# Fagear/SDVPCMdecoder

Hardware: NVIDIA B200
Metric: decoded video lines/sec (bin+CRC+deint) (higher is better)
Workload: dtype u8

## Files before the change

sdvpcmdecoder_b200/csrc/sdv_kernels.cu:

```cuda
#include <cuda_runtime.h>
#include <stdio.h>
#include <new>
#include <vector>
#include <algorithm>
#include "stc007_chain.cuh"
#include "stc007_deint.cuh"
#include "stc007_stitch_host.h"
#include "stc007_bulk.cuh"
#include <unordered_map>
#include <mutex>
#include <chrono>
#include "pcm1_deint.cuh"
#include "pcm16x0_deint.cuh"
#include "pcm1_kernels.cuh"
#include "pcm1_stitch.cuh"
#include "pcm16x0_kernels.cuh"
#include "pcm16x0_stitch.cuh"
#include "pcm16x0_stitch_host.h"

namespace sdv {

__constant__ u16 c_crc_bit[112];
__constant__ u16 c_crc_zero;

struct FastPos { int p0, p1, p2, p3; u32 t0, t1, t2, t3; };

__device__ __forceinline__ FastPos make_fast_pos(Coord coords, int W, int lane)
{
    FastPos f;
    Ppb ppb = make_ppb(coords);
    f.p0 = pixel_of_bit(ppb, lane, 0, W-1);
    f.p1 = pixel_of_bit(ppb, lane+32, 0, W-1);
    f.p2 = pixel_of_bit(ppb, lane+64, 0, W-1);
// ... 298 lines not shown
{
    AsmMap map; long long n_blocks;
    DeintCfg cfg;
    sdv_block_rec *blocks; i16 *samples; u8 *sflags;
    u32 *broken_bits;
    u8 *broken_sum;
    long long tile_base; int tile_stride, tile_len, n_tiles, atomic_bits;
};

__device__ __forceinline__ void block_store(const Block &blk, bool unsafe, long long b, sdv_block_rec *blocks, i16 *samples, u8 *sflags)
{
    if(samples||sflags)
    {
        i16 smp[6]; u8 fl[6];
        blk_output(&blk, smp, fl);
        u32 f03, f45;
        blk_output_flags(&blk, &f03, &f45);
        if(samples)
        {
            u32 *d = (u32 *)(samples+b*6);
            d[0] = (u32)(u16)smp[0]|((u32)(u16)smp[1]<<16); d[1] = (u32)(u16)smp[2]|((u32)(u16)smp[3]<<16); d[2] = (u32)(u16)smp[4]|((u32)(u16)smp[5]<<16);
        }
        if(sflags)
        {
            u16 *d = (u16 *)(sflags+b*6);
            d[0] = (u16)f03; d[1] = (u16)(f03>>16); d[2] = (u16)f45;
        }
    }
    if(blocks) blk_export(&blk, unsafe, blocks+b);
}

enum { DEINT_WARPS = 8, DEINT_TILE = 128, DEINT_TLINES = DEINT_TILE+112, DEINT_THREADS = DEINT_WARPS*32, DEINT_CTA_BLOCKS = DEINT_WARPS*DEINT_TILE };

__global__ void __launch_bounds__(DEINT_THREADS) stc007_deint_kernel(DeintParams p)
{
    __shared__ u16 s_wall[DEINT_WARPS][8][DEINT_TLINES];
    const int warp = threadIdx.x>>5, lane = threadIdx.x&31;
    u16 (*s_w)[DEINT_TLINES] = s_wall[warp];
    const long long tile = (long long)blockIdx.x*DEINT_WARPS+warp;
    if(tile>=p.n_tiles) return;
    const long long b0 = p.tile_base+tile*p.tile_stride;
    if(b0>=p.n_blocks) return;
    int fld0 = 0, j0 = 0;
    const int n_fields = (int)p.map.n_fields, lpf = p.map.lpf, hf = p.map.hf;
    if(p.map.geo)
    {
        const int a0 = (int)b0-p.map.lead_in;
        const int q = (a0>=0) ? (a0/lpf) : -((-a0+lpf-1)/lpf);
        fld0 = q;
        j0 = a0-q*lpf;
    }
    const bool two_fields = p.map.geo&&(lpf>=DEINT_TLINES);
    const sdv_line_rec *fp[2] = { 0, 0 }; int fn[2] = { 0, 0 };
    if(two_fields)
    {
#pragma unroll
        for(int q=0;q<2;q++)
        {
            const int fld = fld0+q;
            if(fld<0) continue;
            if(fld<n_fields) { fp[q] = p.map.recs+((unsigned long long)(u32)(fld>>1)*(u32)p.map.H+(u32)((fld&1)*hf)); fn[q] = hf; }
            else if(p.map.halo&&(fld==n_fields)) { fp[q] = p.map.halo; fn[q] = (hf<112) ? hf : 112; }
        }
    }
    u32 okw[(DEINT_TLINES+31)/32];
    auto line_ptr = [&](int ln) -> const sdv_line_rec *
    {
        if(ln>=DEINT_TLINES) return 0;
        if(!p.map.geo) return (b0+ln<p.map.n_lines) ? (p.map.recs+b0+ln) : (const sdv_line_rec *)0;
        if(two_fields)
        {
            int j = j0+ln;
            const int q = (j>=lpf) ? 1 : 0;
            j -= q ? lpf : 0;
            return (j<(q ? fn[1] : fn[0])) ? ((q ? fp[1] : fp[0])+j) : (const sdv_line_rec *)0;
        }
        int j = j0+ln, fld = fld0;
        while(j>=lpf) { j -= lpf; fld++; }
        if((fld<0)||(j>=hf)) return 0;
        if(fld>=n_fields) return (p.map.halo&&(fld==n_fields)&&(j<112)) ? (p.map.halo+j) : (const sdv_line_rec *)0;
        return p.map.recs+((unsigned long long)(u32)(fld>>1)*(u32)p.map.H+(u32)((fld&1)*hf+j));
    };
    enum { DEINT_GROUP = 4 };
#pragma unroll
    for(int g=0;g<(DEINT_TLINES+31)/32;g+=DEINT_GROUP)
    {
        const sdv_line_rec *r[DEINT_GROUP];
        uint4 wv[DEINT_GROUP], tv[DEINT_GROUP];
#pragma unroll
        for(int i=0;i<DEINT_GROUP;i++) r[i] = line_ptr(lane+32*(g+i));
#pragma unroll
        for(int i=0;i<DEINT_GROUP;i++)
        {
            wv[i] = make_uint4(0, 0, 0, 0); tv[i] = make_uint4(0, 0, 0, 0);
            if(r[i]) { wv[i] = __ldg((const uint4 *)r[i]); tv[i] = __ldg((const uint4 *)r[i]+1); }
        }
#pragma unroll
        for(int i=0;i<DEINT_GROUP;i++)
        {
            const int ln = lane+32*(g+i);
            const uint4 t = tv[i];
            const u32 fl = t.x>>16;
            bool ok = false;
            if(r[i]&&(((t.w>>8)&0xFFu)==SDV_SRV_NO))
            {
                if(!p.cfg.ignore_crc) ok = (fl&SDV_LF_CRC_OK)!=0;
                else { Coord cc; cc.start = (i16)(t.z&0xFFFFu); cc.stop = (i16)(t.z>>16); ok = coord_valid(cc)&&((fl&SDV_LF_BW_SET)!=0); }
            }
            if(ln<DEINT_TLINES)
            {
                s_w[0][ln] = (u16)wv[i].x; s_w[1][ln] = (u16)(wv[i].x>>16); s_w[2][ln] = (u16)wv[i].y; s_w[3][ln] = (u16)(wv[i].y>>16);
                s_w[4][ln] = (u16)wv[i].z; s_w[5][ln] = (u16)(wv[i].z>>16); s_w[6][ln] = (u16)wv[i].w; s_w[7][ln] = (u16)(wv[i].w>>16);
            }
            okw[g+i] = __ballot_sync(0xFFFFFFFFu, ok);
        }
    }
    __syncwarp();
    for(int jt=0;jt<DEINT_TILE/32;jt++)
    {
        const int s = lane+32*jt;
        const long long b = b0+s;
        bool broken_ns = false;
        if((b<p.n_blocks)&&(s<p.tile_len))
        {
            BlockIn in; in.ok = 0;
#pragma unroll
            for(int k=0;k<8;k++)
            {
                const int ln = s+16*k;
                in.w[k] = s_w[k][ln]; in.sw[k] = s_w[7][ln];
                const u32 win = (k&1) ? __funnelshift_r(okw[k>>1], okw[(k>>1)+1], 16) : okw[k>>1];
                in.ok |= (u8)(((win>>lane)&1u)<<k);
            }
            Block blk;
            deint_dispatch(&blk, &in, p.cfg);
            broken_ns = (blk.audio_state==SDV_AUD_BROKEN)&&!blk_silent(&blk);
            block_store(blk, false, b, p.blocks, p.samples, p.sflags);
        }
        const u32 bal = __ballot_sync(0xFFFFFFFFu, broken_ns);
        if(p.atomic_bits)
        {
            if(broken_ns&&p.broken_bits) { atomicOr(&p.broken_bits[b>>5], 1u<<(u32)(b&31)); p.broken_sum[b>>10] = 1; }
        }
        else if((lane==0)&&(b<p.n_blocks))
        {
            if(p.broken_bits) p.broken_bits[b>>5] = bal;
            if(bal&&p.broken_sum) p.broken_sum[b>>10] = 1;
        }
#pragma unroll
        for(int i=0;i+1<(DEINT_TLINES+31)/32;i++) okw[i] = okw[i+1];
    }
}

struct StitchDeintParams
{
    StitchMap map; long long n_blocks;
    DeintCfg cfg;
    sdv_block_rec *blocks; i16 *samples; u8 *sflags;
    u32 *broken_bits; u8 *broken_sum;
};
__global__ void __launch_bounds__(256) stc007_stitch_deint_kernel(StitchDeintParams p)
{
    const long long b = (long long)blockIdx.x*256+threadIdx.x;
    bool broken_ns = false;
    if(b<p.n_blocks)
    {
        int hint = (int)((b-p.map.n_carry-p.map.lead)/p.map.frame_len);
        BlockIn in;
        DeintCfg cfg = p.cfg;
        const bool masked = stitch_block_in(p.map, b, p.cfg.ignore_crc!=0, &in, &hint, &cfg.res_mode);
        Block blk;
        deint_dispatch(&blk, &in, cfg);
        const bool silent = blk_silent(&blk);
        bool unsafe = false;
        if(masked&&!silent) { unsafe = (blk.audio_state!=SDV_AUD_BROKEN); blk_mark_unsafe(&blk); }
        broken_ns = (blk.audio_state==SDV_AUD_BROKEN)&&(!silent)&&(!masked);
        block_store(blk, unsafe, b, p.blocks, p.samples, p.sflags);
    }
    const u32 bal = __ballot_sync(0xFFFFFFFFu, broken_ns);
    if(((threadIdx.x&31)==0)&&(b<p.n_blocks))
    {
        p.broken_bits[b>>5] = bal;
        if(bal) p.broken_sum[b>>10] = 1;
    }
// ... 619 lines not shown
int sdv_bin_decode_frames(sdv_handle *h, const sdv_bin_config *cfg, const uint8_t *luma_dev, int n_frames, int H, int W,
                          int stride, sdv_line_rec *recs_dev, sdv_line_aux *aux_dev, void *cuda_stream)
{
    if(!h) return SDV_ERR_ARG;
    h->first_frame_called = 0;
    const int rc = decode_frames_impl(h, cfg, luma_dev, n_frames, H, W, stride, recs_dev, aux_dev, cuda_stream);
    if((rc==SDV_OK)&&h->first_frame_fn&&!h->first_frame_called) { h->first_frame_called = 1; h->first_frame_fn(h->first_frame_user); }
    return rc;
}

static int decode_frames_impl(sdv_handle *h, const sdv_bin_config *cfg, const uint8_t *luma_dev, int n_frames, int H, int W,
                              int stride, sdv_line_rec *recs_dev, sdv_line_aux *aux_dev, void *cuda_stream)
{
    if(!h) return SDV_ERR_ARG;
    if(!cfg||(n_frames<0)||(H<2)||(H&1)||(H>SDV_MAX_H)||(W<BITS_IN_LINE)||(W>SDV_MAX_W)||(stride<W))
        return fail(h, SDV_ERR_ARG, "sdv_bin_decode_frames: frame geometry (2 <= H <= 1250 even, 137 <= W <= 2048, stride >= W)", cudaSuccess);
    if((n_frames>0)&&(!luma_dev||!recs_dev||((uintptr_t)recs_dev%16)||((uintptr_t)aux_dev%16)))
        return fail(h, SDV_ERR_ARG, "sdv_bin_decode_frames: null or misaligned buffer (records need 16-byte alignment)", cudaSuccess);
    if((cfg->pcm_type!=SDV_TYPE_STC007)&&(cfg->pcm_type!=SDV_TYPE_PCM1)&&(cfg->pcm_type!=SDV_TYPE_PCM16X0)&&(cfg->pcm_type!=SDV_TYPE_M2))
        return fail(h, SDV_ERR_UNSUPPORTED, "pcm_type", cudaSuccess);
    const int dup_flags = (cfg->check_line_dup ? 1 : 0)|((cfg->pcm_type==SDV_TYPE_M2) ? 2 : 0);
    if(cfg->mode>SDV_MODE_INSANE) return fail(h, SDV_ERR_ARG, "mode", cudaSuccess);
    CK(cudaSetDevice(h->device));
    if(h->lazy_pending) return fail(h, SDV_ERR_ARG, "sdv_bin_decode_frames: the previous call was lazy (reserved[2] bit 1): call sdv_bin_decode_verify first", cudaSuccess);
    { const int frc = apply_fine(h); if(frc) return frc; }
    cudaStream_t st = (cudaStream_t)cuda_stream;
    memset(&h->stats, 0, sizeof(h->stats));
    h->stats.lines_total = (uint64_t)n_frames*H;
    if(n_frames==0) return SDV_OK;
    if((cfg->pcm_type==SDV_TYPE_PCM1)||(cfg->pcm_type==SDV_TYPE_PCM16X0)) return p1_decode_frames(h, cfg, luma_dev, n_frames, H, W, stride, recs_dev, aux_dev, st);
    { int rc = ensure(h, (void **)&h->clean, &h->clean_cap, 2*(size_t)n_frames+16); if(rc) return rc; }


    const u32 copy_bytes = (u32)((W+15)&~15);
    int use_tma = (((size_t)stride%16)==0)&&((((uintptr_t)luma_dev)%16)==0);
    u32 slot_bytes = use_tma ? (u32)stride : (((copy_bytes/16)&1) ? copy_bytes : (copy_bytes+16));
    int bulk_warps = (int)((size_t)(227*1024-BULK_SMEM_HEADER)/((size_t)BULK_STAGES*BULK_ROWS*slot_bytes));
    if((bulk_warps<1)&&use_tma)
    {
        use_tma = 0; slot_bytes = ((copy_bytes/16)&1) ? copy_bytes : (copy_bytes+16);
        bulk_warps = (int)((size_t)(227*1024-BULK_SMEM_HEADER)/((size_t)BULK_STAGES*BULK_ROWS*slot_bytes));
    }
    if(bulk_warps>BULK_MAX_WARPS) bulk_warps = BULK_MAX_WARPS;
    if(bulk_warps<1) return fail(h, SDV_ERR_ARG, "line too wide for the bulk kernel", cudaSuccess);
    const size_t bulk_smem = BULK_SMEM_HEADER+(size_t)bulk_warps*BULK_STAGES*BULK_ROWS*slot_bytes;

    int segments = (int)cfg->reserved[0]|((int)cfg->reserved[1]<<8);
    if(segments>n_frames) segments = n_frames;
    if(segments>1)
    {
        h->fuse_arm.armed = 0; h->fuse_done.valid = 0;
        if(h->seg_cap<(size_t)segments)
        {
            cudaFree(h->seg_ctx); h->seg_ctx = NULL; h->seg_cap = 0;
            CK(cudaMalloc(&h->seg_ctx, (size_t)segments*sizeof(ChainCtx)));
            h->seg_cap = (size_t)segments;
        }
        ChainParams cp; memset(&cp, 0, sizeof(cp));
        cp.luma = luma_dev; cp.H = H; cp.W = W; cp.stride = (size_t)stride;
        cp.f_begin = 0; cp.n_frames = n_frames; cp.max_frames = n_frames;
        cp.recs = recs_dev; cp.aux = aux_dev; cp.ctx = h->seg_ctx;
        cp.clean = NULL; cp.have_spec = 0; cp.spec_ref = 0; cp.spec_coords = coord_none();
        cp.reset = 1; cp.mode = cfg->mode; cp.line_dup = dup_flags; cp.segments = segments;
        stc007_chain_kernel<256><<<segments, 256, 0, st>>>(cp);
        h->stats.kernel_launches++;
        CK(cudaStreamSynchronize(st));
        CK(cudaGetLastError());
        h->stats.lines_chain = h->stats.lines_total;
        h->acc_launches += h->stats.kernel_launches;
        return SDV_OK;
    }

    const bool cont = (cfg->reserved[3]&1)&&h->chain_open&&(h->chain_H==H)&&(h->chain_W==W)&&(h->chain_mode==(cfg->mode|(dup_flags<<8)));
    if((cfg->reserved[3]&1)&&!cont) return fail(h, SDV_ERR_ARG, "sdv_bin_decode_frames: nothing to continue (no earlier call with this geometry and mode on the handle)", cudaSuccess);
    h->chain_open = 0;
    int f = 0;
    bool have_spec = false; u8 spec_ref = 0, spec_black = 0, spec_white = 0; Coord spec_c = coord_none();
    uint64_t frames_bulk = 0;
    const bool fuse_req = h->fuse_arm.armed&&(cfg->pcm_type==SDV_TYPE_STC007)&&(H/2<=BULK_FUSE_HF)&&(H/2<=h->fuse_arm.geo.lines_per_field)&&!cont;
    h->fuse_arm.armed = 0; h->fuse_done.valid = 0;
    int fuse_launches = 0, fuse_from = 0; bool fuse_ok = fuse_req;
    DeintScratch fsc; memset(&fsc, 0, sizeof(fsc));
    long long fuse_blocks = 0;
    if(fuse_req)
    {
        fuse_blocks = (long long)h->fuse_arm.geo.lead_in+(long long)n_frames*2*h->fuse_arm.geo.lines_per_field;
        const int rc = deint_scratch(h, fuse_blocks, h->fuse_arm.cfg.broken_mask_dur, &fsc);
        if(rc) return rc;
    }

    static const int bulk_blocks_env = getenv("SDV_BULK_BLOCKS") ? atoi(getenv("SDV_BULK_BLOCKS")) : 0;
    const int bulk_blocks = (bulk_blocks_env>0) ? ((bulk_blocks_env<h->num_sms) ? bulk_blocks_env : h->num_sms)
                                                : ((h->num_sms>8) ? (h->num_sms*88)/100 : h->num_sms);
    auto launch_bulk = [&](cudaStream_t bst, int f_from, const BinState &b, int *first_unclean_dev)
    {
        BulkParams bp;
        bp.luma = luma_dev; bp.H = H; bp.W = W; bp.stride = (size_t)stride;
        bp.f0 = f_from; bp.n_frames = n_frames-f_from;
        bp.ref = b.def_ref; bp.black = b.def_black; bp.white = b.def_white; bp.line_dup = (u8)dup_flags; bp.coords = b.def_coord;
        bp.recs = recs_dev; bp.aux = aux_dev; bp.clean = h->clean; bp.first_unclean = first_unclean_dev;
        bp.use_tma = use_tma; bp.copy_bytes = copy_bytes; bp.slot_bytes = slot_bytes; bp.warps = bulk_warps;
        { const Ppb ppb = make_ppb(b.def_coord); for(int i=0;i<BITS_PCM_DATA;i++) bp.pos[i] = (u32)pixel_of_bit(ppb, i, 0, W-1); }
        const long long units = (long long)(n_frames-f_from);
        const bool fuse = fuse_req&&(fuse_launches==0);
        int warps = bulk_warps; size_t smem = bulk_smem;
        if(fuse)
        {
            warps = (int)((size_t)(227*1024-BULK_SMEM_HEADER)/((size_t)BULK_STAGES*BULK_ROWS*slot_bytes+BULK_FUSE_BYTES));
            if(warps>BULK_MAX_WARPS) warps = BULK_MAX_WARPS;
            if(warps<1) { fuse_ok = false; warps = bulk_warps; }
            else smem = BULK_SMEM_HEADER+(size_t)warps*((size_t)BULK_STAGES*BULK_ROWS*slot_bytes+BULK_FUSE_BYTES);
        }
        const bool fuse_now = fuse&&fuse_ok;
        bp.warps = warps;
        bp.samples = NULL; bp.sflags = NULL; bp.broken_bits = NULL; bp.broken_sum = NULL; bp.block0 = 0; bp.lpf = 0;
        if(fuse_now)
        {
            bp.samples = h->fuse_arm.samples; bp.sflags = h->fuse_arm.sflags;
            bp.broken_bits = fsc.bits; bp.broken_sum = fsc.sum;
            bp.block0 = h->fuse_arm.geo.lead_in; bp.lpf = h->fuse_arm.geo.lines_per_field;
            cudaMemsetAsync(fsc.bits, 0, (size_t)((fuse_blocks+31)>>5)*sizeof(u32)+(size_t)((fuse_blocks+1023)>>10), bst);
            fuse_from = f_from;
        }
        else if(fuse_req) fuse_ok = false;
        fuse_launches++;
        int grid = (int)((units+warps-1)/warps);
        const int max_blocks = (fuse_now&&(bulk_blocks_env<=0)&&(h->num_sms>8)) ? (h->num_sms-1) : bulk_blocks;
        if(grid>max_blocks) grid = max_blocks;
        timing_flush(h, 0);
        cudaEventRecord(h->ev[0], bst);
        if(fuse_now) stc007_bulk_kernel<true><<<grid, warps*32, smem, bst>>>(bp);
        else stc007_bulk_kernel<false><<<grid, warps*32, smem, bst>>>(bp);
        cudaEventRecord(h->ev[1], bst);
        h->ev_set[0] = 1; h->ev_units[0] = (uint64_t)(n_frames-f_from)*(uint64_t)H;
        h->stats.kernel_launches++;
    };

    bool warm_pending = false;
    if(h->warm_valid&&(h->warm_H==H)&&(h->warm_W==W)&&(h->warm_mode==(cfg->mode|(dup_flags<<8)))&&(n_frames>1)&&!(cfg->reserved[2]&1))
    {
        CK(cudaEventRecord(h->ev_sync[0], st));
        CK(cudaStreamWaitEvent(h->copy_stream, h->ev_sync[0], 0));
        set_int_kernel<<<1, 1, 0, h->copy_stream>>>(h->spec_fu, n_frames);
        launch_bulk(h->copy_stream, 1, h->warm_bin, h->spec_fu);
        CK(cudaEventRecord(h->ev_sync[1], h->copy_stream));
        warm_pending = true;
    }
    enum { RELAY_AFTER = 2, RELAY_MIN_FRAMES = 32, RELAY_WARM = 2, RELAY_LEN = 2, CHAIN_LAUNCH_FRAMES = 64 };
    int chain_run = 0;
    bool relayed = false;
    int relay_end = 0, relay_pieces = 0, relay_redone = 0;
    auto relay_decode = [&](int f0) -> int
    {
        static const int len_env = getenv("SDV_RELAY_LEN") ? atoi(getenv("SDV_RELAY_LEN")) : 0;
        const int len = (len_env>0) ? len_env : RELAY_LEN;
        const int span = (n_frames-f0<4*h->num_sms*len) ? (n_frames-f0) : (4*h->num_sms*len);
        const int left = span;
        const int pieces = (left+len-1)/len;
        const int n_frames_all = n_frames;
        const int n_frames = f0+span;
        (void)n_frames_all;
        relay_end = n_frames;
        int rc;
        if(h->seg_cap<(size_t)pieces)
        {
            cudaFree(h->seg_ctx); h->seg_ctx = NULL; h->seg_cap = 0;
            CK(cudaMalloc(&h->seg_ctx, (size_t)pieces*sizeof(ChainCtx)));
            h->seg_cap = (size_t)pieces;
        }
        if((rc = ensure(h, (void **)&h->start_ctx, &h->start_cap, (size_t)pieces*sizeof(ChainCtx)))) return rc;
        if((rc = ensure(h, (void **)&h->fmed, &h->fmed_cap, 2*(size_t)n_frames_all*sizeof(Coord)))) return rc;
        if((rc = ensure(h, (void **)&h->snaps, &h->snaps_cap, (size_t)n_frames_all*sizeof(ChainSnap)))) return rc;
        if((rc = ensure(h, (void **)&h->warm_scratch, &h->warm_cap, (size_t)pieces*CHAIN_BATCH*sizeof(sdv_line_rec)))) return rc;
        if((rc = ensure(h, (void **)&h->relay_ok, &h->relay_ok_cap, (size_t)pieces*(1+sizeof(int))+32))) return rc;
        if(h->relay_ok_host_cap<(size_t)pieces)
        {
            cudaFreeHost(h->relay_ok_host); h->relay_ok_host = NULL; h->relay_ok_host_cap = 0;
// ... 84 lines not shown
        bool warm_hit = false;
        if(warm_pending)
        {
            warm_pending = false;
            const BinState &wb = h->warm_bin, &cb = h->hdr_host->bin;
            warm_hit = (f==1)&&h->hdr_host->stable&&(wb.def_ref==cb.def_ref)&&coord_eq(wb.def_coord, cb.def_coord)
                       &&(wb.def_black==cb.def_black)&&(wb.def_white==cb.def_white);
            if(warm_hit&&h->first_frame_fn&&!h->first_frame_called)
            {
                h->first_frame_called = 1;
                h->first_frame_fn(h->first_frame_user);
            }
            CK(cudaStreamWaitEvent(st, h->ev_sync[1], 0));
            if(!warm_hit)
            {
                CK(cudaStreamSynchronize(st));
                h->warm_valid = 0;
                if(fuse_req) h->fuse_arm.armed = 1;
                return decode_frames_impl(h, cfg, luma_dev, n_frames, H, W, stride, recs_dev, aux_dev, cuda_stream);
            }
            have_spec = true; spec_ref = wb.def_ref; spec_c = wb.def_coord; spec_black = wb.def_black; spec_white = wb.def_white;
        }
        if(f>=n_frames) break;
        if(!h->hdr_host->stable)
        {
            chain_run += f-f_launch;
            continue;
        }
        chain_run += f-f_launch;
        const BinState b = h->hdr_host->bin;
        bool bulk_ran = warm_hit;
        if(!have_spec||(spec_ref!=b.def_ref)||!coord_eq(spec_c, b.def_coord))
        {
            launch_bulk(st, f, b, &h->ctx->first_unclean);
            have_spec = true; spec_ref = b.def_ref; spec_c = b.def_coord; spec_black = b.def_black; spec_white = b.def_white;
            bulk_ran = true;
        }
        if(!bulk_ran)
        {
            first_unclean_kernel<<<1, 1024, 0, st>>>(h->clean, f, n_frames, h->ctx);
            h->stats.kernel_launches++;
        }
        int fb;
        if(warm_hit&&(cfg->reserved[2]&2)&&!cont)
        {
            if((b.def_black!=spec_black)||(b.def_white!=spec_white))
            {
                const size_t cnt = (size_t)(n_frames-f)*H;
                patch_bw_kernel<<<(unsigned)((cnt+255)/256), 256, 0, st>>>(recs_dev, (size_t)f*H, cnt, b.def_black, b.def_white);
                h->stats.kernel_launches++;
            }
            chain_skip_dev_kernel<<<1, 1, 0, st>>>(h->ctx, h->spec_fu, f);
            h->stats.kernel_launches++;
            CK(cudaMemcpyAsync(h->fu_host, h->spec_fu, sizeof(int), cudaMemcpyDeviceToHost, st));
            CK(cudaEventRecord(h->ev_lazy, st));
            h->lazy_pending = 1; h->lazy_cfg = *cfg; h->lazy_luma = luma_dev; h->lazy_n = n_frames; h->lazy_H = H; h->lazy_W = W; h->lazy_stride = stride;
            h->lazy_recs = recs_dev; h->lazy_aux = aux_dev; h->lazy_stream = cuda_stream;
            frames_bulk += (uint64_t)(n_frames-f);
            f = n_frames;
            break;
        }
        if(warm_hit)
        {
            CK(cudaMemcpyAsync(h->fu_host, h->spec_fu, sizeof(int), cudaMemcpyDeviceToHost, st));
            CK(cudaStreamSynchronize(st));
            fb = *h->fu_host;
        }
// ... 100 lines not shown
}

static int run_deint(sdv_handle *h, const sdv_deint_config *cfg, const AsmMap &map, long long n_blocks,
                     sdv_block_rec *blocks_dev, int16_t *samples_dev, uint8_t *sample_flags_dev, cudaStream_t st)
{
    if(n_blocks<=0) return SDV_OK;
    if(cfg->cwd) return fail(h, SDV_ERR_UNSUPPORTED, "CWD needs the stitcher's frame queue: use sdv_stc007_stitch_frames (sdv_deint_config.cwd)", cudaSuccess);
    DeintScratch sc;
    { int rc = deint_scratch(h, n_blocks, cfg->broken_mask_dur, &sc); if(rc) return rc; }
    DeintParams p;
    p.map = map; p.n_blocks = n_blocks;
    p.cfg = make_deint_cfg(cfg);
    p.blocks = blocks_dev; p.samples = samples_dev; p.sflags = sample_flags_dev;
    const bool windows = cfg->broken_mask_dur>0;
    p.broken_bits = windows ? sc.bits : NULL; p.broken_sum = windows ? sc.sum : NULL;
    p.tile_base = 0; p.tile_stride = DEINT_TILE; p.tile_len = DEINT_TILE; p.atomic_bits = 0;
    p.n_tiles = (int)((n_blocks+DEINT_TILE-1)/DEINT_TILE);
    const auto &fd = h->fuse_done;
    const bool fused = fd.valid&&map.geo&&(!blocks_dev)&&(samples_dev==fd.samples)&&(sample_flags_dev==fd.sflags)&&(map.recs==fd.recs)
                       &&(map.lead_in==fd.lead_in)&&(map.lpf==fd.lpf)&&(map.H==fd.H)&&(map.n_fields==2*(long long)fd.n_frames)&&(cfg->broken_mask_dur==fd.dur)
                       &&deint_cfg_is_std14(p.cfg)&&(!p.cfg.ignore_crc)&&(!p.cfg.m2)&&windows;
    h->fuse_done.valid = 0;
    timing_flush(h, 1);
    cudaEventRecord(h->ev[2], st);
    if(fused)
    {
        p.atomic_bits = 1;
        const long long head = (long long)fd.lead_in+(long long)fd.f_from*2*fd.lpf;
        if(head>0)
        {
            DeintParams q = p;
            q.n_blocks = (head<n_blocks) ? head : n_blocks;
            q.n_tiles = (int)((q.n_blocks+DEINT_TILE-1)/DEINT_TILE);
            stc007_deint_kernel<<<(unsigned)((q.n_tiles+DEINT_WARPS-1)/DEINT_WARPS), DEINT_THREADS, 0, st>>>(q);
            h->acc_launches += 1;
        }
        const int n_rest = fd.n_frames-fd.f_from;
        if(n_rest>0)
        {
            DeintParams q = p;
            q.tile_base = head+(2*fd.lpf-112); q.tile_stride = 2*fd.lpf; q.tile_len = 112; q.n_tiles = n_rest;
            stc007_deint_kernel<<<(unsigned)((q.n_tiles+DEINT_WARPS-1)/DEINT_WARPS), DEINT_THREADS, 0, st>>>(q);
            h->acc_launches += 1;
        }
    }
    else
    {
        if(windows) CK(cudaMemsetAsync(sc.sum, 0, (size_t)((n_blocks+1023)>>10), st));
        const unsigned grid = (unsigned)((n_blocks+DEINT_CTA_BLOCKS-1)/DEINT_CTA_BLOCKS);
        stc007_deint_kernel<<<grid, DEINT_THREADS, 0, st>>>(p);
        h->acc_launches += 1;
    }
    cudaEventRecord(h->ev[3], st);
    h->ev_set[1] = 1; h->ev_units[1] = (uint64_t)n_blocks;
    if(windows)
    {
        WindowParams wp; memset(&wp, 0, sizeof(wp));
        wp.stitched = 0; wp.amap = map; wp.n_blocks = n_blocks; wp.cfg = p.cfg;
        wp.blocks = blocks_dev; wp.samples = samples_dev; wp.sflags = sample_flags_dev;
        int rc = run_windows(h, sc, wp, cfg->broken_mask_dur, cfg->countdown_in, st);
        if(rc) return rc;
    }
    CK(cudaGetLastError());
    return SDV_OK;
}

int sdv_stc007_fuse_next_decode(sdv_handle *h, const sdv_deint_config *cfg, const sdv_stc007_geometry *geo, int16_t *samples_dev, uint8_t *sample_flags_dev)
{
    if(!h) return SDV_ERR_ARG;
    h->fuse_arm.armed = 0;
    if(!cfg||!geo||!samples_dev||!sample_flags_dev||((uintptr_t)samples_dev%4)||((uintptr_t)sample_flags_dev%2))
        return fail(h, SDV_ERR_ARG, "sdv_stc007_fuse_next_decode: null or misaligned buffers", cudaSuccess);
    const DeintCfg c = make_deint_cfg(cfg);
    if(!deint_cfg_is_std14(c)||c.ignore_crc||c.m2||cfg->cwd||(cfg->broken_mask_dur==0)||(geo->lines_per_field<120))
        return SDV_OK;
    h->fuse_arm.armed = 1; h->fuse_arm.cfg = *cfg; h->fuse_arm.geo = *geo; h->fuse_arm.samples = samples_dev; h->fuse_arm.sflags = sample_flags_dev;
    return SDV_OK;
}

int sdv_stc007_countdown_copy(sdv_handle *h, int32_t *state_dev, void *cuda_stream)
{
    if(!h||!state_dev) return SDV_ERR_ARG;
    CK(cudaSetDevice(h->device));
// ... 766 lines not shown
```

sdvpcmdecoder_b200/csrc/stc007_bulk.cuh:

```cuda
#pragma once
#include "stc007_chain.cuh"
#include "stc007_deint.cuh"

namespace sdv {

__constant__ u16 c_crc8[3*256];
enum { BULK_SMEM_HEADER = 128+3*512 };

__device__ __forceinline__ u32 smem_u32(const void *p) { return (u32)__cvta_generic_to_shared(p); }
__device__ __forceinline__ void mbar_init(u64 *bar, int count)
{
    asm volatile("mbarrier.init.shared::cta.b64 [%0], %1;" :: "r"(smem_u32(bar)), "r"(count));
}
__device__ __forceinline__ void mbar_expect_tx(u64 *bar, u32 bytes)
{
    asm volatile("mbarrier.arrive.expect_tx.shared::cta.b64 _, [%0], %1;" :: "r"(smem_u32(bar)), "r"(bytes) : "memory");
}
__device__ __forceinline__ void mbar_wait(u64 *bar, u32 parity)
{
    u32 done;
    do
    {
        asm volatile("{\n .reg .pred p;\n mbarrier.try_wait.parity.shared::cta.b64 p, [%1], %2;\n selp.u32 %0, 1, 0, p;\n}"
                     : "=r"(done) : "r"(smem_u32(bar)), "r"(parity) : "memory");
    }
    while(!done);
}
__device__ __forceinline__ void bulk_g2s(u32 dst_smem, const void *src, u32 bytes, u64 *bar)
{
    asm volatile("cp.async.bulk.shared::cluster.global.mbarrier::complete_tx::bytes [%0], [%1], %2, [%3];"
                 :: "r"(dst_smem), "l"(src), "r"(bytes), "r"(smem_u32(bar)) : "memory");
}

struct BulkParams
{
    const u8 *luma; int H, W; size_t stride;
    int f0, n_frames;
    u8 ref, black, white, line_dup; Coord coords;
    sdv_line_rec *recs; sdv_line_aux *aux;
    u8 *clean;
    int *first_unclean;
    int use_tma, warps; u32 copy_bytes, slot_bytes;
    u32 pos[BITS_PCM_DATA];
    i16 *samples; u8 *sflags;
    u32 *broken_bits; u8 *broken_sum;
    long long block0;
    int lpf;
};
enum { BULK_FUSE_HF = 288, BULK_FUSE_BYTES = 2*8*BULK_FUSE_HF*2+2*BULK_FUSE_HF };

template<int OFF, int LEN>
__device__ __forceinline__ u32 stream_field(u32 b0, u32 b1, u32 b2, u32 b3)
{
    constexpr int idx = OFF>>5, sh = 32-(OFF&31)-LEN;
    const u32 hi = (idx==0) ? b0 : ((idx==1) ? b1 : ((idx==2) ? b2 : b3));
    const u32 lo = (idx==0) ? b1 : ((idx==1) ? b2 : ((idx==2) ? b3 : 0u));
    constexpr u32 mask = (1u<<LEN)-1u;
    if constexpr (sh>=0) return (hi>>sh)&mask;
    else return __funnelshift_l(lo, hi, (u32)(-sh))&mask;
}

__device__ __forceinline__ void resolve_equal_cells(u32 *g, const u32 *ge)
{
    u32 gr[4], er[4];
#pragma unroll
    for(int i=0;i<4;i++) { gr[i] = __brev(g[i]); er[i] = __brev(ge[i]&~g[i]); }
    u64 alo = ((u64)(gr[1]|er[1])<<32)|(gr[0]|er[0]), ahi = ((u64)(gr[3]|er[3])<<32)|(gr[2]|er[2]);
    u64 blo = ((u64)gr[1]<<32)|gr[0], bhi = ((u64)gr[3]<<32)|gr[2];
    u64 slo = alo+blo;
    u64 cy = (slo<alo) ? 1ull : 0ull;
    u64 shi = ahi+bhi+cy;
    u64 cout = ((shi<ahi)||(cy&&(shi==ahi))) ? 1ull : 0ull;
    u64 clo = slo^alo^blo, chi = shi^ahi^bhi;
    u64 rlo = (clo>>1)|(chi<<63), rhi = (chi>>1)|(cout<<63);
    g[0] = __brev((u32)rlo); g[1] = __brev((u32)(rlo>>32)); g[2] = __brev((u32)rhi); g[3] = __brev((u32)(rhi>>32));
}

__device__ __forceinline__ bool packed_almost_silent(u32 w01, u32 w23, u32 w45)
{
    const u32 a = ((w01+0x00040004u)&0x3FF83FF8u), b = ((w23+0x00040004u)&0x3FF83FF8u), c = ((w45+0x00040004u)&0x3FF83FF8u);
    const int cnt = ((a&0xFFFFu)==0)+((a>>16)==0)+((b&0xFFFFu)==0)+((b>>16)==0)+((c&0xFFFFu)==0)+((c>>16)==0);
    return cnt>=2;
}
__device__ __forceinline__ int packed_diff8(u32 a01, u32 a23, u32 a45, u32 a67, u32 b01, u32 b23, u32 b45, u32 b67)
{
    const u32 m = 0x00FF00FFu;
    return __popc((a01^b01)&m)+__popc((a23^b23)&m)+__popc((a45^b45)&m)+__popc((a67^b67)&m);
}
__device__ __forceinline__ bool packed_control_block(u32 w01, u32 w23, u32 w45, u32 w67)
{
    return (w01==0x0CCC3333u)&&(w23==0x0CCC3333u)&&((w45&0xFFFFu)==0)&&(((w67>>16)&0x0FF0u)==0);
}

enum { BULK_MAX_WARPS = 4, BULK_STAGES = 2, BULK_ROWS = 32 };

template<bool FUSE>
__global__ void __launch_bounds__(BULK_MAX_WARPS*32, 1) stc007_bulk_kernel(const __grid_constant__ BulkParams p)
{
    extern __shared__ __align__(128) u8 dsm[];
    u64 *bars = (u64 *)dsm;
    u16 *crc_tab = (u16 *)(dsm+128);
    const int warp = threadIdx.x>>5, lane = threadIdx.x&31;
    const u32 stage_bytes = BULK_ROWS*p.slot_bytes;
    u8 *ring = dsm+BULK_SMEM_HEADER+(size_t)warp*BULK_STAGES*stage_bytes;
    u64 *bar = bars+warp*BULK_STAGES;
    u16 *fw = (u16 *)(dsm+BULK_SMEM_HEADER+(size_t)p.warps*BULK_STAGES*stage_bytes+(size_t)warp*BULK_FUSE_BYTES);
    u8 *fok = (u8 *)(fw+2*8*BULK_FUSE_HF);
    for(int i=threadIdx.x;i<3*256;i+=blockDim.x) crc_tab[i] = c_crc8[i];
    if(p.use_tma&&(lane==0))
    {
        for(int s=0;s<BULK_STAGES;s++) mbar_init(&bar[s], 1);
        asm volatile("fence.mbarrier_init.release.cluster;" ::: "memory");
    }
    __syncthreads();

    const int hf = p.H/2;
    const int nbatch = (p.H+BULK_ROWS-1)/BULK_ROWS;
    const long long n_units = p.n_frames;
    const long long gw = (long long)blockIdx.x*p.warps+warp, gstride = (long long)gridDim.x*p.warps;
    const long long my_units = (gw<n_units) ? ((n_units-gw+gstride-1)/gstride) : 0;
    const long long n_items = my_units*nbatch;
    const int ref = p.ref;
    const int fld = lane&1;

    auto issue = [&](long long it)
    {
        const long long u = gw+(it/nbatch)*gstride;
        const int r0 = (int)(it%nbatch)*BULK_ROWS;
        const int rows = (p.H-r0<BULK_ROWS) ? (p.H-r0) : BULK_ROWS;
        const int s = (int)(it&1);
        if(lane==0)
        {
            const u32 bytes = (u32)rows*(u32)p.stride;
            mbar_expect_tx(&bar[s], bytes);
            bulk_g2s(smem_u32(ring)+(u32)s*stage_bytes, p.luma+((size_t)(p.f0+u)*p.H+(size_t)r0)*p.stride, bytes, &bar[s]);
        }
        __syncwarp();
    };
    if(p.use_tma) { if(n_items>0) issue(0); if(n_items>1) issue(1); }

    u32 c01 = 0, c23 = 0, c45 = 0, c67 = 0;
    bool c_cb = false;
    u32 frame_bad = 0;
    const u32 rec5 = (u32)p.ref|((u32)p.black<<8)|((u32)p.white<<16);
    const u32 rec6 = (u32)(u16)p.coords.start|((u32)(u16)p.coords.stop<<16);

    for(long long it=0;it<n_items;it++)
    {
        const long long u = gw+(it/nbatch)*gstride;
        const int b = (int)(it%nbatch), r0 = b*BULK_ROWS;
        const int rows = (p.H-r0<BULK_ROWS) ? (p.H-r0) : BULK_ROWS;
        const int f = p.f0+(int)u;
        const int s = (int)(it&1);
        const int k = (r0>>1)+(lane>>1);
        const bool active = lane<rows;
        const u8 *row = ring+(size_t)s*stage_bytes+(size_t)lane*p.slot_bytes;
        if(p.use_tma) mbar_wait(&bar[s], (u32)((it>>1)&1));
        else
        {
            __syncwarp();
            for(int r=0;r<rows;r++)
            {
                const u8 *src = p.luma+((size_t)f*p.H+(size_t)(r0+r))*p.stride;
                u8 *dst = ring+(size_t)s*stage_bytes+(size_t)r*p.slot_bytes;
                for(int j=lane;j<p.W;j+=32) dst[j] = __ldg(src+j);
            }
            __syncwarp();
        }
        u32 g[4], ge[4];
#pragma unroll
        for(int w=0;w<4;w++)
        {
            u32 a = 0, c = 0;
#pragma unroll
            for(int j=0;j<32;j++)
            {
                const int v = row[p.pos[32*w+j]];
                a = __funnelshift_l((u32)(ref-v), a, 1);
                c = __funnelshift_l((u32)(ref-1-v), c, 1);
            }
            g[w] = a; ge[w] = c;
        }
        __syncwarp();
        if(p.use_tma&&(it+BULK_STAGES<n_items)) issue(it+BULK_STAGES);
        const bool any_eq = ((ge[0]^g[0])|(ge[1]^g[1])|(ge[2]^g[2])|(ge[3]^g[3]))!=0;
        if(__any_sync(0xFFFFFFFFu, any_eq)) resolve_equal_cells(g, ge);
        const u32 w0 = stream_field<0, 14>(g[0], g[1], g[2], g[3]), w1 = stream_field<14, 14>(g[0], g[1], g[2], g[3]);
        const u32 w2 = stream_field<28, 14>(g[0], g[1], g[2], g[3]), w3 = stream_field<42, 14>(g[0], g[1], g[2], g[3]);
        const u32 w4 = stream_field<56, 14>(g[0], g[1], g[2], g[3]), w5 = stream_field<70, 14>(g[0], g[1], g[2], g[3]);
        const u32 w6 = stream_field<84, 14>(g[0], g[1], g[2], g[3]), w7 = stream_field<98, 14>(g[0], g[1], g[2], g[3]);
        u32 w8 = g[3]&0xFFFFu;
        u32 crc_a = 0xFFFFu, crc_b = 0;
#pragma unroll
        for(int j=0;j<7;j++)
        {
            const u32 ma = (g[j>>2]>>(24-8*(j&3)))&0xFFu, mb = (g[(j+7)>>2]>>(24-8*((j+7)&3)))&0xFFu;
            crc_a = ((crc_a<<8)^crc_tab[((crc_a>>8)^ma)&0xFFu])&0xFFFFu;
            crc_b = ((crc_b<<8)^crc_tab[((crc_b>>8)^mb)&0xFFu])&0xFFFFu;
// ... 120 lines not shown
```

Baseline: 8.107 billion.

## Load only the PCM pixel window via TMA tensor maps and add a specialized standard deinterleave kernel

The bulk binarization pass now computes the horizontal pixel window that actually holds PCM bits and fetches only that window with a 2D TMA tensor copy, where it used to copy whole rows with a 1D bulk copy. This cuts global-to-shared traffic and shared memory per warp, and the per-block warp cap rises from 4 to 6. The deinterleave kernel gains a templated fast path for standard 14-bit configs that packs the line-valid bit into the high bit of each stored word instead of keeping ballot bitmaps, and writes samples and flags directly. The price is a driver entry point lookup, tensor map encoding on the host, and a second kernel instantiation. The full-row-height expect_tx relies on TMA counting the full box bytes when the last batch runs past the tensor's edge.

```diff
diff --git a/sdvpcmdecoder_b200/csrc/sdv_kernels.cu b/sdvpcmdecoder_b200/csrc/sdv_kernels.cu
--- a/sdvpcmdecoder_b200/csrc/sdv_kernels.cu
+++ b/sdvpcmdecoder_b200/csrc/sdv_kernels.cu
@@ -1,4 +1,5 @@
 #include <cuda_runtime.h>
+#include <cudaTypedefs.h>
 #include <stdio.h>
 #include <new>
 #include <vector>
@@ -363,6 +364,7 @@
 
 enum { DEINT_WARPS = 8, DEINT_TILE = 128, DEINT_TLINES = DEINT_TILE+112, DEINT_THREADS = DEINT_WARPS*32, DEINT_CTA_BLOCKS = DEINT_WARPS*DEINT_TILE };
 
+template<bool STD>
 __global__ void __launch_bounds__(DEINT_THREADS) stc007_deint_kernel(DeintParams p)
 {
     __shared__ u16 s_wall[DEINT_WARPS][8][DEINT_TLINES];
@@ -394,7 +396,7 @@
             else if(p.map.halo&&(fld==n_fields)) { fp[q] = p.map.halo; fn[q] = (hf<112) ? hf : 112; }
         }
     }
-    u32 okw[(DEINT_TLINES+31)/32];
+    u32 okw[STD ? 1 : (DEINT_TLINES+31)/32];
     auto line_ptr = [&](int ln) -> const sdv_line_rec *
     {
         if(ln>=DEINT_TLINES) return 0;
@@ -438,12 +440,18 @@
                 if(!p.cfg.ignore_crc) ok = (fl&SDV_LF_CRC_OK)!=0;
                 else { Coord cc; cc.start = (i16)(t.z&0xFFFFu); cc.stop = (i16)(t.z>>16); ok = coord_valid(cc)&&((fl&SDV_LF_BW_SET)!=0); }
             }
+            uint4 w = wv[i];
+            if(STD)
+            {
+                const u32 okb = ok ? 0x80008000u : 0u;
+                w.x = (w.x&0x3FFF3FFFu)|okb; w.y = (w.y&0x3FFF3FFFu)|okb; w.z = (w.z&0x3FFF3FFFu)|okb; w.w = (w.w&0x3FFF3FFFu)|okb;
+            }
             if(ln<DEINT_TLINES)
             {
-                s_w[0][ln] = (u16)wv[i].x; s_w[1][ln] = (u16)(wv[i].x>>16); s_w[2][ln] = (u16)wv[i].y; s_w[3][ln] = (u16)(wv[i].y>>16);
-                s_w[4][ln] = (u16)wv[i].z; s_w[5][ln] = (u16)(wv[i].z>>16); s_w[6][ln] = (u16)wv[i].w; s_w[7][ln] = (u16)(wv[i].w>>16);
+                s_w[0][ln] = (u16)w.x; s_w[1][ln] = (u16)(w.x>>16); s_w[2][ln] = (u16)w.y; s_w[3][ln] = (u16)(w.y>>16);
+                s_w[4][ln] = (u16)w.z; s_w[5][ln] = (u16)(w.z>>16); s_w[6][ln] = (u16)w.w; s_w[7][ln] = (u16)(w.w>>16);
             }
-            okw[g+i] = __ballot_sync(0xFFFFFFFFu, ok);
+            if(!STD) okw[g+i] = __ballot_sync(0xFFFFFFFFu, ok);
         }
     }
     __syncwarp();
@@ -452,7 +460,34 @@
         const int s = lane+32*jt;
         const long long b = b0+s;
         bool broken_ns = false;
-        if((b<p.n_blocks)&&(s<p.tile_len))
+        if(STD)
+        {
+            if((b<p.n_blocks)&&(s<p.tile_len))
+            {
+                BlockIn in; in.ok = 0;
+#pragma unroll
+                for(int k=0;k<8;k++)
+                {
+                    const u32 v = s_w[k][s+16*k];
+                    in.w[k] = (u16)(v&0x3FFFu);
+                    in.ok |= (u8)((v>>15)<<k);
+                }
+                Block blk;
+                deint_block_std14(&blk, &in);
+                blk.m2 = 0;
+                u32 f03, f45;
+                blk_output_flags(&blk, &f03, &f45);
+                const u32 s01 = (((u32)blk.words[0]<<2)&0xFFFFu)|((u32)blk.words[1]<<18);
+                const u32 s23 = (((u32)blk.words[2]<<2)&0xFFFFu)|((u32)blk.words[3]<<18);
+                const u32 s45 = (((u32)blk.words[4]<<2)&0xFFFFu)|((u32)blk.words[5]<<18);
+                u32 *ds = (u32 *)(p.samples+b*6);
+                u16 *df = (u16 *)(p.sflags+b*6);
+                ds[0] = s01; ds[1] = s23; ds[2] = s45;
+                df[0] = (u16)f03; df[1] = (u16)(f03>>16); df[2] = (u16)f45;
+                broken_ns = (blk.audio_state==SDV_AUD_BROKEN)&&!blk_silent(&blk);
+            }
+        }
+        else if((b<p.n_blocks)&&(s<p.tile_len))
         {
             BlockIn in; in.ok = 0;
 #pragma unroll
@@ -478,9 +513,18 @@
             if(p.broken_bits) p.broken_bits[b>>5] = bal;
             if(bal&&p.broken_sum) p.broken_sum[b>>10] = 1;
         }
+        if(!STD)
+        {
 #pragma unroll
-        for(int i=0;i+1<(DEINT_TLINES+31)/32;i++) okw[i] = okw[i+1];
-    }
+            for(int i=0;i+1<(DEINT_TLINES+31)/32;i++) okw[i] = okw[i+1];
+        }
+    }
+}
+
+static void launch_deint(const DeintParams &p, unsigned grid, cudaStream_t st)
+{
+    if(deint_cfg_is_std14(p.cfg)&&!p.cfg.m2&&!p.blocks&&p.samples&&p.sflags) stc007_deint_kernel<true><<<grid, DEINT_THREADS, 0, st>>>(p);
+    else stc007_deint_kernel<false><<<grid, DEINT_THREADS, 0, st>>>(p);
 }
 
 struct StitchDeintParams
@@ -1166,18 +1210,20 @@
     { int rc = ensure(h, (void **)&h->clean, &h->clean_cap, 2*(size_t)n_frames+16); if(rc) return rc; }
 
 
-    const u32 copy_bytes = (u32)((W+15)&~15);
-    int use_tma = (((size_t)stride%16)==0)&&((((uintptr_t)luma_dev)%16)==0);
-    u32 slot_bytes = use_tma ? (u32)stride : (((copy_bytes/16)&1) ? copy_bytes : (copy_bytes+16));
-    int bulk_warps = (int)((size_t)(227*1024-BULK_SMEM_HEADER)/((size_t)BULK_STAGES*BULK_ROWS*slot_bytes));
-    if((bulk_warps<1)&&use_tma)
-    {
-        use_tma = 0; slot_bytes = ((copy_bytes/16)&1) ? copy_bytes : (copy_bytes+16);
-        bulk_warps = (int)((size_t)(227*1024-BULK_SMEM_HEADER)/((size_t)BULK_STAGES*BULK_ROWS*slot_bytes));
-    }
-    if(bulk_warps>BULK_MAX_WARPS) bulk_warps = BULK_MAX_WARPS;
-    if(bulk_warps<1) return fail(h, SDV_ERR_ARG, "line too wide for the bulk kernel", cudaSuccess);
-    const size_t bulk_smem = BULK_SMEM_HEADER+(size_t)bulk_warps*BULK_STAGES*BULK_ROWS*slot_bytes;
+    const int use_tma = (((size_t)stride%16)==0)&&((((uintptr_t)luma_dev)%16)==0);
+    PFN_cuTensorMapEncodeTiled_v12000 encode_tiled = NULL;
+    if(use_tma)
+    {
+        static PFN_cuTensorMapEncodeTiled_v12000 fn = NULL;
+        if(!fn)
+        {
+            void *ptr = NULL; cudaDriverEntryPointQueryResult qr;
+            CK(cudaGetDriverEntryPointByVersion("cuTensorMapEncodeTiled", &ptr, 12000, cudaEnableDefault, &qr));
+            if(qr!=cudaDriverEntryPointSuccess) return fail(h, SDV_ERR_CUDA, "cuTensorMapEncodeTiled not found in the driver", cudaSuccess);
+            fn = (PFN_cuTensorMapEncodeTiled_v12000)ptr;
+        }
+        encode_tiled = fn;
+    }
 
     int segments = (int)cfg->reserved[0]|((int)cfg->reserved[1]<<8);
     if(segments>n_frames) segments = n_frames;
@@ -1233,15 +1279,36 @@
         bp.f0 = f_from; bp.n_frames = n_frames-f_from;
         bp.ref = b.def_ref; bp.black = b.def_black; bp.white = b.def_white; bp.line_dup = (u8)dup_flags; bp.coords = b.def_coord;
         bp.recs = recs_dev; bp.aux = aux_dev; bp.clean = h->clean; bp.first_unclean = first_unclean_dev;
-        bp.use_tma = use_tma; bp.copy_bytes = copy_bytes; bp.slot_bytes = slot_bytes; bp.warps = bulk_warps;
-        { const Ppb ppb = make_ppb(b.def_coord); for(int i=0;i<BITS_PCM_DATA;i++) bp.pos[i] = (u32)pixel_of_bit(ppb, i, 0, W-1); }
+        int pmin = W, pmax = 0;
+        {
+            const Ppb ppb = make_ppb(b.def_coord);
+            for(int i=0;i<BITS_PCM_DATA;i++) { const int x = pixel_of_bit(ppb, i, 0, W-1); bp.pos[i] = (u32)x; pmin = std::min(pmin, x); pmax = std::max(pmax, x); }
+        }
+        bp.x_lo = pmin&~15; bp.win_bytes = (u32)(((pmax+16)&~15)-bp.x_lo);
+        for(int i=0;i<BITS_PCM_DATA;i++) bp.pos[i] -= (u32)bp.x_lo;
+        const u32 slot_bytes = (use_tma||((bp.win_bytes/16)&1)) ? bp.win_bytes : (bp.win_bytes+16);
+        bp.use_tma = use_tma; bp.slot_bytes = slot_bytes;
+        int bulk_warps = (int)((size_t)(227*1024-BULK_SMEM_HEADER)/((size_t)BULK_STAGES*BULK_ROWS*slot_bytes));
+        if(bulk_warps>STC_BULK_MAX_WARPS) bulk_warps = STC_BULK_MAX_WARPS;
+        { static const int wenv = getenv("SDV_BULK_WARPS") ? atoi(getenv("SDV_BULK_WARPS")) : 0; if((wenv>0)&&(wenv<bulk_warps)) bulk_warps = wenv; }
+        memset(&bp.tmap, 0, sizeof(bp.tmap));
+        if(use_tma)
+        {
+            const cuuint64_t gdim[2] = { (cuuint64_t)((W+7)/8), (cuuint64_t)n_frames*(cuuint64_t)H };
+            const cuuint64_t gstride[1] = { (cuuint64_t)stride };
+            const cuuint32_t box[2] = { bp.win_bytes/8, BULK_ROWS }, estride[2] = { 1, 1 };
+            const CUresult r = encode_tiled(&bp.tmap, CU_TENSOR_MAP_DATA_TYPE_UINT64, 2, (void *)luma_dev, gdim, gstride, box, estride,
+                                            CU_TENSOR_MAP_INTERLEAVE_NONE, CU_TENSOR_MAP_SWIZZLE_NONE, CU_TENSOR_MAP_L2_PROMOTION_L2_256B,
+                                            CU_TENSOR_MAP_FLOAT_OOB_FILL_NONE);
+            if(r!=CUDA_SUCCESS) return fail(h, SDV_ERR_CUDA, "cuTensorMapEncodeTiled (bulk pass window)", cudaSuccess);
+        }
         const long long units = (long long)(n_frames-f_from);
         const bool fuse = fuse_req&&(fuse_launches==0);
-        int warps = bulk_warps; size_t smem = bulk_smem;
+        int warps = bulk_warps; size_t smem = BULK_SMEM_HEADER+(size_t)bulk_warps*BULK_STAGES*BULK_ROWS*slot_bytes;
         if(fuse)
         {
             warps = (int)((size_t)(227*1024-BULK_SMEM_HEADER)/((size_t)BULK_STAGES*BULK_ROWS*slot_bytes+BULK_FUSE_BYTES));
-            if(warps>BULK_MAX_WARPS) warps = BULK_MAX_WARPS;
+            if(warps>STC_BULK_MAX_WARPS) warps = STC_BULK_MAX_WARPS;
             if(warps<1) { fuse_ok = false; warps = bulk_warps; }
             else smem = BULK_SMEM_HEADER+(size_t)warps*((size_t)BULK_STAGES*BULK_ROWS*slot_bytes+BULK_FUSE_BYTES);
         }
@@ -1268,6 +1335,7 @@
         cudaEventRecord(h->ev[1], bst);
         h->ev_set[0] = 1; h->ev_units[0] = (uint64_t)(n_frames-f_from)*(uint64_t)H;
         h->stats.kernel_launches++;
+        return (int)SDV_OK;
     };
 
     bool warm_pending = false;
@@ -1276,7 +1344,7 @@
         CK(cudaEventRecord(h->ev_sync[0], st));
         CK(cudaStreamWaitEvent(h->copy_stream, h->ev_sync[0], 0));
         set_int_kernel<<<1, 1, 0, h->copy_stream>>>(h->spec_fu, n_frames);
-        launch_bulk(h->copy_stream, 1, h->warm_bin, h->spec_fu);
+        { const int rc = launch_bulk(h->copy_stream, 1, h->warm_bin, h->spec_fu); if(rc) return rc; }
         CK(cudaEventRecord(h->ev_sync[1], h->copy_stream));
         warm_pending = true;
     }
@@ -1427,7 +1495,7 @@
         bool bulk_ran = warm_hit;
         if(!have_spec||(spec_ref!=b.def_ref)||!coord_eq(spec_c, b.def_coord))
         {
-            launch_bulk(st, f, b, &h->ctx->first_unclean);
+            { const int rc = launch_bulk(st, f, b, &h->ctx->first_unclean); if(rc) return rc; }
             have_spec = true; spec_ref = b.def_ref; spec_c = b.def_coord; spec_black = b.def_black; spec_white = b.def_white;
             bulk_ran = true;
         }
@@ -1594,7 +1662,7 @@
             DeintParams q = p;
             q.n_blocks = (head<n_blocks) ? head : n_blocks;
             q.n_tiles = (int)((q.n_blocks+DEINT_TILE-1)/DEINT_TILE);
-            stc007_deint_kernel<<<(unsigned)((q.n_tiles+DEINT_WARPS-1)/DEINT_WARPS), DEINT_THREADS, 0, st>>>(q);
+            launch_deint(q, (unsigned)((q.n_tiles+DEINT_WARPS-1)/DEINT_WARPS), st);
             h->acc_launches += 1;
         }
         const int n_rest = fd.n_frames-fd.f_from;
@@ -1602,7 +1670,7 @@
         {
             DeintParams q = p;
             q.tile_base = head+(2*fd.lpf-112); q.tile_stride = 2*fd.lpf; q.tile_len = 112; q.n_tiles = n_rest;
-            stc007_deint_kernel<<<(unsigned)((q.n_tiles+DEINT_WARPS-1)/DEINT_WARPS), DEINT_THREADS, 0, st>>>(q);
+            launch_deint(q, (unsigned)((q.n_tiles+DEINT_WARPS-1)/DEINT_WARPS), st);
             h->acc_launches += 1;
         }
     }
@@ -1610,7 +1678,7 @@
     {
         if(windows) CK(cudaMemsetAsync(sc.sum, 0, (size_t)((n_blocks+1023)>>10), st));
         const unsigned grid = (unsigned)((n_blocks+DEINT_CTA_BLOCKS-1)/DEINT_CTA_BLOCKS);
-        stc007_deint_kernel<<<grid, DEINT_THREADS, 0, st>>>(p);
+        launch_deint(p, grid, st);
         h->acc_launches += 1;
     }
     cudaEventRecord(h->ev[3], st);
diff --git a/sdvpcmdecoder_b200/csrc/stc007_bulk.cuh b/sdvpcmdecoder_b200/csrc/stc007_bulk.cuh
--- a/sdvpcmdecoder_b200/csrc/stc007_bulk.cuh
+++ b/sdvpcmdecoder_b200/csrc/stc007_bulk.cuh
@@ -1,4 +1,5 @@
 #pragma once
+#include <cuda.h>
 #include "stc007_chain.cuh"
 #include "stc007_deint.cuh"
 
@@ -31,16 +32,23 @@
     asm volatile("cp.async.bulk.shared::cluster.global.mbarrier::complete_tx::bytes [%0], [%1], %2, [%3];"
                  :: "r"(dst_smem), "l"(src), "r"(bytes), "r"(smem_u32(bar)) : "memory");
 }
+__device__ __forceinline__ void tensor2d_g2s(u32 dst_smem, const CUtensorMap *map, int x, int y, u64 *bar)
+{
+    asm volatile("cp.async.bulk.tensor.2d.shared::cluster.global.mbarrier::complete_tx::bytes [%0], [%1, {%2, %3}], [%4];"
+                 :: "r"(dst_smem), "l"((unsigned long long)map), "r"(x), "r"(y), "r"(smem_u32(bar)) : "memory");
+}
 
 struct BulkParams
 {
+    CUtensorMap tmap;
     const u8 *luma; int H, W; size_t stride;
     int f0, n_frames;
     u8 ref, black, white, line_dup; Coord coords;
     sdv_line_rec *recs; sdv_line_aux *aux;
     u8 *clean;
     int *first_unclean;
-    int use_tma, warps; u32 copy_bytes, slot_bytes;
+    int use_tma, warps; u32 slot_bytes;
+    int x_lo; u32 win_bytes;
     u32 pos[BITS_PCM_DATA];
     i16 *samples; u8 *sflags;
     u32 *broken_bits; u8 *broken_sum;
@@ -93,9 +101,10 @@
 }
 
 enum { BULK_MAX_WARPS = 4, BULK_STAGES = 2, BULK_ROWS = 32 };
+enum { STC_BULK_MAX_WARPS = 6 };
 
 template<bool FUSE>
-__global__ void __launch_bounds__(BULK_MAX_WARPS*32, 1) stc007_bulk_kernel(const __grid_constant__ BulkParams p)
+__global__ void __launch_bounds__(STC_BULK_MAX_WARPS*32, 1) stc007_bulk_kernel(const __grid_constant__ BulkParams p)
 {
     extern __shared__ __align__(128) u8 dsm[];
     u64 *bars = (u64 *)dsm;
@@ -127,13 +136,11 @@
     {
         const long long u = gw+(it/nbatch)*gstride;
         const int r0 = (int)(it%nbatch)*BULK_ROWS;
-        const int rows = (p.H-r0<BULK_ROWS) ? (p.H-r0) : BULK_ROWS;
         const int s = (int)(it&1);
         if(lane==0)
         {
-            const u32 bytes = (u32)rows*(u32)p.stride;
-            mbar_expect_tx(&bar[s], bytes);
-            bulk_g2s(smem_u32(ring)+(u32)s*stage_bytes, p.luma+((size_t)(p.f0+u)*p.H+(size_t)r0)*p.stride, bytes, &bar[s]);
+            mbar_expect_tx(&bar[s], stage_bytes);
+            tensor2d_g2s(smem_u32(ring)+(u32)s*stage_bytes, &p.tmap, p.x_lo/8, (int)((p.f0+u)*p.H+r0), &bar[s]);
         }
         __syncwarp();
     };
@@ -159,11 +166,12 @@
         else
         {
             __syncwarp();
+            const int n = ((p.W-p.x_lo)<(int)p.win_bytes) ? (p.W-p.x_lo) : (int)p.win_bytes;
             for(int r=0;r<rows;r++)
             {
-                const u8 *src = p.luma+((size_t)f*p.H+(size_t)(r0+r))*p.stride;
+                const u8 *src = p.luma+((size_t)f*p.H+(size_t)(r0+r))*p.stride+p.x_lo;
                 u8 *dst = ring+(size_t)s*stage_bytes+(size_t)r*p.slot_bytes;
-                for(int j=lane;j<p.W;j+=32) dst[j] = __ldg(src+j);
+                for(int j=lane;j<n;j+=32) dst[j] = __ldg(src+j);
             }
             __syncwarp();
         }
```

After: 7.749 billion (median of 6 runs). 0.956x the previous value.
